# noamteyssier/ibu

Measured on AMD Instinct MI355X. Metric: records/s, fused 2-bit decode+encode of 24-byte IBU records (HBM-resident), higher is better.
Workload: dtype u64

## Files before the change

### ibu_amd/csrc/k_encode.hip

```cpp
#include "kcommon.hpp"
#include "kernels.h"

namespace ibu {

#ifndef IBU_ENCODE_MINWAVES
#define IBU_ENCODE_MINWAVES 6
#endif
#ifndef IBU_ENCODE_GEN_MINWAVES
#define IBU_ENCODE_GEN_MINWAVES 4
#endif
constexpr int encode_minwaves(int bc, int um) {
  if (bc == 0 || um == 0) return IBU_ENCODE_GEN_MINWAVES;
  return (bc <= 16 && um <= 16) ? IBU_ENCODE_MINWAVES : 4;
}
__host__ __device__ constexpr u32 enc_field_lds(int spec_len, u32 len) { return spec_len > 0 ? 128u * len : 32u * len + kStreamPad; }
template <int BC, int UM>
constexpr int enc_nt() {
#ifdef IBU_ENCODE_NT
  return (BC > 0 && UM > 0 && (BC & 3) == 0 && (UM & 3) == 0) ? IBU_ENCODE_NT : 1;
#else
  return 1;
#endif
}
#ifndef IBU_ENCODE_NT2_MINWAVES
#define IBU_ENCODE_NT2_MINWAVES 5
#endif
template <int BC, int UM>
constexpr int enc_waves() { return enc_nt<BC, UM>() > 1 ? IBU_ENCODE_NT2_MINWAVES : encode_minwaves(BC, UM); }

template <int BC, int UM, bool MSB>
__global__ void __launch_bounds__(kBlock, (enc_waves<BC, UM>()))
ibu_k_encode(const uint8_t* __restrict__ bc_in, const uint8_t* __restrict__ umi_in,
             const u64* __restrict__ idx_in, u64 first_index, u64 row_base, u32 ntiles, u32 bc_len, u32 umi_len,
             u32 wave_lds_bytes, uint8_t* __restrict__ recs, u64* __restrict__ status) {
  constexpr int NT = enc_nt<BC, UM>(), kRecs = kTileRecs * NT;
  extern __shared__ __attribute__((aligned(16))) uint8_t dyn_lds[];
  const u32 lane = threadIdx.x & (kWave - 1);
  const u32 wib = threadIdx.x >> 6;
  if (BC > 0) bc_len = BC;
  if (UM > 0) umi_len = UM;
  uint8_t* area = dyn_lds + wib * wave_lds_bytes;
  uint8_t* asc_bc = area;
  uint8_t* asc_umi = area + enc_field_lds(BC, bc_len) * NT;
  const TileRange tr = tile_range(ntiles, wib);
  const u32 nwaves = tr.stride;
  u32 t = tr.t;
  ntiles = tr.end;
  if (t >= ntiles) return;
  const uint8_t* idx_src = idx_in ? reinterpret_cast<const uint8_t*>(idx_in) + 16 * lane : bc_in;
  const size_t idx_tile = idx_in ? 1024 * NT : 0, idx_sub = idx_in ? 1024 : 0;

  AsciiStage<BC, NT> sb;
  AsciiStage<UM, NT> su;
  u32x4 vi[NT];
  sb.issue(bc_in + (size_t)t * kRecs * bc_len, bc_len, lane);
  su.issue(umi_in + (size_t)t * kRecs * umi_len, umi_len, lane);
#pragma unroll
  for (int j = 0; j < NT; ++j) vi[j] = ld16(idx_src + (size_t)t * idx_tile + j * idx_sub);
  BadRows bad;
  for (;;) {
    const size_t row0 = (size_t)t * kRecs;
    wave_lds_fence();
    const bool okcb = sb.land(asc_bc, bc_len, lane), okcu = su.land(asc_umi, umi_len, lane);
    const bool chunks_ok = okcb && okcu;
    u64 ix[NT][2];
#pragma unroll
    for (int j = 0; j < NT; ++j) {
      ix[j][0] = ((u64)vi[j].y << 32) | vi[j].x;
      ix[j][1] = ((u64)vi[j].w << 32) | vi[j].z;
      if (!idx_in) { ix[j][0] = first_index + row0 + 128 * j + 2 * lane; ix[j][1] = ix[j][0] + 1; }
    }
    const u32 tn = t + nwaves;
    const bool more = tn < ntiles;
    const u32 tp = more ? tn : t;
    sb.issue(bc_in + (size_t)tp * kRecs * bc_len, bc_len, lane);
    su.issue(umi_in + (size_t)tp * kRecs * umi_len, umi_len, lane);
#pragma unroll
    for (int j = 0; j < NT; ++j) vi[j] = ld16(idx_src + (size_t)tp * idx_tile + j * idx_sub);
    wave_lds_fence();
    u64 b[NT][2], u[NT][2];
#pragma unroll
    for (int j = 0; j < NT; ++j)
#pragma unroll
      for (int h = 0; h < 2; ++h) {
        const u32 r = 128 * j + 2 * lane + h;
        bool okb = true, oku = true;
#if IBU_PROBE == 1
        b[j][h] = *reinterpret_cast<const u32*>(asc_bc + r * bc_len);
        u[j][h] = *reinterpret_cast<const u32*>(asc_umi + r * umi_len);
#elif IBU_PROBE == 2
        b[j][h] = row0 + r;
        u[j][h] = b[j][h] * 3;
#else
        b[j][h] = pack_row<BC>(asc_bc, r, bc_len, okb);
        u[j][h] = pack_row<UM>(asc_umi, r, umi_len, oku);
        if constexpr (BC == 0 || UM == 0) {
          if (__ballot(!chunks_ok) != 0) {
            if constexpr (BC == 0) b[j][h] = pack_row_bytes(bc_in + (row0 + r) * bc_len, bc_len, okb);
            if constexpr (UM == 0) u[j][h] = pack_row_bytes(umi_in + (row0 + r) * umi_len, umi_len, oku);
          }
        }
#endif
        if (!okb) b[j][h] = 0;
        if (!oku) u[j][h] = 0;
        bad.note(!(okb && oku), row_base + row0 + r);
      }
    wave_lds_fence();
#pragma unroll
    for (int j = 0; j < NT; ++j) {
      u64* r = reinterpret_cast<u64*>(area + (128 * j + 2 * lane) * 24);
      r[0] = b[j][0]; r[1] = u[j][0]; r[2] = ix[j][0]; r[3] = b[j][1]; r[4] = u[j][1]; r[5] = ix[j][1];
    }
    wave_lds_fence();
    if constexpr (MSB) {
      rev_pairs_tile<NT>(area, 24, 0, bc_len, lane);
      rev_pairs_tile<NT>(area, 24, 8, umi_len, lane);
      wave_lds_fence();
    }
    uint8_t* dst = recs + (size_t)t * (kTileBytes * NT) + 16 * lane;
#pragma unroll
    for (int k = 0; k < 3 * NT; ++k) st16(dst + 1024 * k, *reinterpret_cast<const u32x4*>(area + 1024 * k + 16 * lane));
    if (!more) break;
    t = tn;
  }
  bad.flush(status);
}

constexpr int pack_nt(int len) { return (len > 0 && len <= 16) ? 2 : 1; }
template <int LEN, bool MSB, int GNT = 1, int RND = 0>
__global__ void __launch_bounds__(kBlock, LEN == 0 ? (RND >= 7 ? 5 : (GNT >= 4 || RND >= 5) ? 6 : 8) : LEN <= 12 ? 5 : 4)
ibu_k_pack(const uint8_t* __restrict__ in, u64 row_base, u32 ntiles , u32 len, u64* __restrict__ codes,
           u64* __restrict__ status) {
  constexpr int NT = LEN > 0 ? pack_nt(LEN) : GNT, kRows = kTileRecs * NT;
  constexpr u32 kWaveLds = LEN > 0 ? (u32)(kRows * LEN) : (u32)(256 * (RND > 0 ? RND : 4)) + kStreamPad;
  __shared__ __attribute__((aligned(16))) uint8_t lds[kWavesPerBlock * kWaveLds];
  const u32 lane = threadIdx.x & (kWave - 1);
  const u32 wib = threadIdx.x >> 6;
  uint8_t* asc = lds + wib * kWaveLds;
  const TileRange tr = tile_range(ntiles, wib);
  const u32 nwaves = tr.stride;
  u32 t = tr.t;
  ntiles = tr.end;
  if (LEN > 0) len = LEN;
  if (t >= ntiles) return;
  AsciiStage<LEN, NT, RND> sv;
  sv.issue(in + (size_t)t * kRows * len, len, lane);
  BadRows bad;
  for (;;) {
    const size_t row0 = (size_t)t * kRows;
    wave_lds_fence();
    const bool chunks_ok = sv.land(asc, len, lane);
    const u32 tn = t + nwaves;
    const bool more = tn < ntiles;
    sv.issue(in + (size_t)(more ? tn : t) * kRows * len, len, lane);
    wave_lds_fence();
#pragma unroll
    for (int j = 0; j < NT; ++j) {
      const u32 r = 128 * j + 2 * lane;
      bool ok0 = true, ok1 = true;
      u64 v0 = pack_row<LEN>(asc, r, len, ok0);
      u64 v1 = pack_row<LEN>(asc, r + 1, len, ok1);
      if constexpr (LEN == 0) {
        if (__ballot(!chunks_ok) != 0) {
          v0 = pack_row_bytes(in + (row0 + r) * len, len, ok0);
          v1 = pack_row_bytes(in + (row0 + r + 1) * len, len, ok1);
        }
      }
      if constexpr (MSB) { v0 = rev_pairs(v0, len); v1 = rev_pairs(v1, len); }
      if (!ok0) v0 = 0;
      if (!ok1) v1 = 0;
      bad.note(!ok0, row_base + row0 + r);
      bad.note(!ok1, row_base + row0 + r + 1);
      u32x4 o; o.x = (u32)v0; o.y = (u32)(v0 >> 32); o.z = (u32)v1; o.w = (u32)(v1 >> 32);
      st16(reinterpret_cast<uint8_t*>(codes) + (row0 + 128 * j) * 8 + 16 * lane, o);
    }
    if (!more) break;
    t = tn;
  }
  bad.flush(status);
}

extern "C" __global__ void ibu_k_encode_tail(const uint8_t* bc_in, const uint8_t* umi_in, const u64* idx_in,
                                             u64 first_index, u64 row0, u64 n, u32 bc_len, u32 umi_len, u32 msb,
                                             u64* __restrict__ recs, u64* status) {
  const u64 i = row0 + (u64)blockIdx.x * blockDim.x + threadIdx.x;
  if (i >= n) return;
  bool okb = true, oku = true;
  u64 b = pack_row_bytes(bc_in + i * bc_len, bc_len, okb);
  u64 u = pack_row_bytes(umi_in + i * umi_len, umi_len, oku);
  if (msb) { b = rev_pairs(b, bc_len); u = rev_pairs(u, umi_len); }
  if (!okb) b = 0;
  if (!oku) u = 0;
  if (!(okb && oku)) { atomicMin(&status[0], i); atomicAdd(&status[1], 1ull); }
  recs[3 * i] = b; recs[3 * i + 1] = u; recs[3 * i + 2] = idx_in ? idx_in[i] : first_index + i;
}
extern "C" __global__ void ibu_k_pack_tail(const uint8_t* in, u64 row0, u64 n, u32 len, u32 msb, u64* codes, u64* status) {
  const u64 i = row0 + (u64)blockIdx.x * blockDim.x + threadIdx.x;
  if (i >= n) return;
  bool ok = true;
  u64 v = pack_row_bytes(in + i * len, len, ok);
  if (msb) v = rev_pairs(v, len);
  if (!ok) { v = 0; atomicMin(&status[0], i); atomicAdd(&status[1], 1ull); }
  codes[i] = v;
}

typedef void (*EncFn)(const uint8_t*, const uint8_t*, const u64*, u64, u64, u32, u32, u32, u32, uint8_t*, u64*);
template <int B, int U, bool M>
static constexpr EncFn enc_entry() { return ibu_k_encode<len_of_mode(B), len_of_mode(U), M>; }
#define IBU_ENC_ROW(B, M) {enc_entry<B, 0, M>(), enc_entry<B, 1, M>(), enc_entry<B, 2, M>(), enc_entry<B, 3, M>(), enc_entry<B, 4, M>()}
#define IBU_ENC_TABLE(M) {IBU_ENC_ROW(0, M), IBU_ENC_ROW(1, M), IBU_ENC_ROW(2, M), IBU_ENC_ROW(3, M), IBU_ENC_ROW(4, M)}
static const EncFn kEncTable[2][kNumLenModes][kNumLenModes] = {IBU_ENC_TABLE(false), IBU_ENC_TABLE(true)};
template <int B, int U>
static constexpr int enc_nt_of() { return enc_nt<len_of_mode(B), len_of_mode(U)>(); }
#define IBU_ENC_NT_ROW(B) {enc_nt_of<B, 0>(), enc_nt_of<B, 1>(), enc_nt_of<B, 2>(), enc_nt_of<B, 3>(), enc_nt_of<B, 4>()}
static const int kEncNtTable[kNumLenModes][kNumLenModes] = {IBU_ENC_NT_ROW(0), IBU_ENC_NT_ROW(1), IBU_ENC_NT_ROW(2),
                                                            IBU_ENC_NT_ROW(3), IBU_ENC_NT_ROW(4)};

hipError_t launch_encode(const LaunchCfg& cfg, const uint8_t* bc, const uint8_t* umi, const uint64_t* idx,
                         uint64_t first_index, size_t n, uint32_t bc_len, uint32_t umi_len, void* recs,
                         uint64_t* status, hipStream_t st) {
  (void)hipGetLastError();
  if (n == 0) return hipSuccess;
  const Span sp[4] = {{recs, 24}, {bc, bc_len}, {umi, umi_len}, {idx, 8}};
  const int mb = mode_of_len(bc_len), mu = mode_of_len(umi_len);
  const u32 nt = (u32)kEncNtTable[mb][mu];
  const size_t tile_recs = (size_t)kTileRecs * nt;
  const RowSplit rs = split_rows(cfg, sp, 4, n, tile_recs);
  if (rs.head)
    hipLaunchKernelGGL(ibu_k_encode_tail, dim3(tail_grid(rs.head)), dim3(256), 0, st, bc, umi, (const u64*)idx, (u64)first_index,
                       (u64)0, (u64)rs.head, bc_len, umi_len, cfg.base_order, (u64*)recs, (u64*)status);
  if (rs.main) {
    const u32 ntiles = (u32)(rs.main / tile_recs);
    u32 wave_lds = (enc_field_lds(len_of_mode(mb), bc_len) + enc_field_lds(len_of_mode(mu), umi_len)) * nt;
    if (wave_lds < (u32)kTileBytes * nt) wave_lds = kTileBytes * nt;
    const int mo = cfg.base_order ? 1 : 0;
    const EncFn fn = kEncTable[mo][mb][mu];
    static std::atomic<int> occ[2][33][33];
    const int nb = resident_blocks<kBlock>(cfg, fn, wave_lds * kWavesPerBlock, &occ[mo][bc_len][umi_len]);
    hipLaunchKernelGGL(fn, dim3(grid_for(ntiles, cfg.cus, nb)), dim3(kBlock), wave_lds * kWavesPerBlock, st,
                       adv(bc, rs.head * bc_len), adv(umi, rs.head * umi_len), adv((const u64*)idx, 8 * rs.head),
                       (u64)(first_index + rs.head), (u64)rs.head, ntiles, bc_len, umi_len, wave_lds,
                       adv((uint8_t*)recs, 24 * rs.head), (u64*)status);
  }
  if (rs.head + rs.main < n)
    hipLaunchKernelGGL(ibu_k_encode_tail, dim3(tail_grid(n - rs.head - rs.main)), dim3(256), 0, st, bc, umi, (const u64*)idx,
                       (u64)first_index, (u64)(rs.head + rs.main), (u64)n, bc_len, umi_len, cfg.base_order, (u64*)recs, (u64*)status);
  return hipGetLastError();
}

typedef void (*PackFn)(const uint8_t*, u64, u32, u32, u64*, u64*);
#define IBU_PACK_ROW(M) {nullptr , ibu_k_pack<len_of_mode(1), M>, ibu_k_pack<len_of_mode(2), M>, \
                         ibu_k_pack<len_of_mode(3), M>, ibu_k_pack<len_of_mode(4), M>}
static const PackFn kPackTable[2][kNumLenModes] = {IBU_PACK_ROW(false), IBU_PACK_ROW(true)};
struct PackShape { int nt, rounds; };
static inline PackShape pack_shape(uint32_t len) {
  const int nt = len <= 8 ? 4 : 2;
  return {nt, (int)(len * nt + 7) / 8};
}
template <bool M>
static PackFn pack_gen_entry(int nt, int rounds) {
  switch (nt * 10 + rounds) {
    case 41: return ibu_k_pack<0, M, 4, 1>;
    case 42: return ibu_k_pack<0, M, 4, 2>;
    case 43: return ibu_k_pack<0, M, 4, 3>;
    case 44: return ibu_k_pack<0, M, 4, 4>;
    case 23: return ibu_k_pack<0, M, 2, 3>;
    case 24: return ibu_k_pack<0, M, 2, 4>;
    case 25: return ibu_k_pack<0, M, 2, 5>;
    case 26: return ibu_k_pack<0, M, 2, 6>;
    case 27: return ibu_k_pack<0, M, 2, 7>;
    default: return ibu_k_pack<0, M, 2, 8>;
  }
}

hipError_t launch_pack(const LaunchCfg& cfg, const uint8_t* in, size_t n, uint32_t len, uint64_t* codes,
                       uint64_t* status, hipStream_t st) {
  (void)hipGetLastError();
  if (n == 0) return hipSuccess;
  const Span sp[2] = {{in, len}, {codes, 8}};
  const int m = mode_of_len(len), mo = cfg.base_order ? 1 : 0;
  const PackShape shape = m ? PackShape{pack_nt(len_of_mode(m)), 0} : pack_shape(len);
  const size_t tile_rows = (size_t)kTileRecs * shape.nt;
  const RowSplit rs = split_rows(cfg, sp, 2, n, tile_rows);
  if (rs.head)
    hipLaunchKernelGGL(ibu_k_pack_tail, dim3(tail_grid(rs.head)), dim3(256), 0, st, in, (u64)0, (u64)rs.head, len, cfg.base_order,
                       (u64*)codes, (u64*)status);
  if (rs.main) {
    const u32 ntiles = (u32)(rs.main / tile_rows);
    const PackFn fn = m ? kPackTable[mo][m] : (mo ? pack_gen_entry<true>(shape.nt, shape.rounds) : pack_gen_entry<false>(shape.nt, shape.rounds));
    static std::atomic<int> occ[2][kNumLenModes], occ_gen[2][33];
    std::atomic<int>* oc = m ? &occ[mo][m] : &occ_gen[mo][len];
    hipLaunchKernelGGL(fn, dim3(grid_for(ntiles, cfg.cus, resident_blocks<kBlock>(cfg, fn, 0, oc))),
                       dim3(kBlock), 0, st, adv(in, rs.head * len), (u64)rs.head, ntiles, len, adv((u64*)codes, 8 * rs.head),
                       (u64*)status);
  }
  if (rs.head + rs.main < n)
    hipLaunchKernelGGL(ibu_k_pack_tail, dim3(tail_grid(n - rs.head - rs.main)), dim3(256), 0, st, in, (u64)(rs.head + rs.main),
                       (u64)n, len, cfg.base_order, (u64*)codes, (u64*)status);
  return hipGetLastError();
}

}
```

### ibu_amd/csrc/kcommon.hpp

```cpp
#pragma once
#include <hip/hip_runtime.h>
#include <stdint.h>
#include <stdio.h>
#include <stdlib.h>

#include "kernels.h"

namespace ibu {

typedef unsigned int u32;
typedef unsigned long long u64;
typedef u32 u32x4 __attribute__((ext_vector_type(4)));
typedef u32 u32x2 __attribute__((ext_vector_type(2)));

static constexpr int kWave = 64;
#ifndef IBU_BLOCK
#define IBU_BLOCK 256
#endif
static constexpr int kBlock = IBU_BLOCK;
static constexpr int kWavesPerBlock = kBlock / kWave;
static constexpr int kTileRecs = 128;
static constexpr int kTileBytes = kTileRecs * 24;
static constexpr u32 kPool = 0x54474341u;

static constexpr int kNumLenModes = 5;
__host__ __device__ constexpr int len_of_mode(int m) { return m == 1 ? 8 : m == 2 ? 12 : m == 3 ? 16 : m == 4 ? 32 : 0; }
static inline int mode_of_len(uint32_t len) {
  switch (len) {
    case 8: return 1;
    case 12: return 2;
    case 16: return 3;
    case 32: return 4;
    default: return 0;
  }
}

#ifndef IBU_XCD_REMAP
#define IBU_XCD_REMAP 1
#endif
__device__ __forceinline__ u32 logical_block() {
#if IBU_XCD_REMAP
  const u32 nb = gridDim.x;
  if (nb & 7u) return blockIdx.x;
  return (blockIdx.x & 7u) * (nb >> 3) + (blockIdx.x >> 3);
#else
  return blockIdx.x;
#endif
}

#ifndef IBU_XCD_STATIC
#define IBU_XCD_STATIC 1
#endif
struct TileRange { u32 t, stride, end; };
#ifndef IBU_XCD_SUB
#define IBU_XCD_SUB 1
#endif
__device__ __forceinline__ TileRange tile_range(u32 ntiles, u32 wib) {
#if IBU_XCD_STATIC
  if ((gridDim.x & 7u) == 0 && gridDim.x >= 8u * IBU_XCD_SUB) {
    const u32 parts = 8u * IBU_XCD_SUB;
    const u32 tpp = (ntiles + parts - 1) / parts;
    const u32 xcd = blockIdx.x & 7u, lb = blockIdx.x >> 3, nbx = gridDim.x >> 3;
    const u32 sub = lb % IBU_XCD_SUB, part = xcd * IBU_XCD_SUB + sub;
    const u32 nb_sub = (nbx - sub + IBU_XCD_SUB - 1) / IBU_XCD_SUB;
    const u32 t0 = part * tpp, t1 = t0 + tpp < ntiles ? t0 + tpp : ntiles;
    return {t0 + (lb / IBU_XCD_SUB) * (u32)kWavesPerBlock + wib, nb_sub * (u32)kWavesPerBlock, t0 < ntiles ? t1 : 0u};
  }
#endif
  return {logical_block() * (u32)kWavesPerBlock + wib, gridDim.x * (u32)kWavesPerBlock, ntiles};
}

template <class Regs, class Load, class Body>
__device__ __forceinline__ void sweep_tiles(const TileRange tr, Load load, Body body) {
  u32 t = tr.t;
  if (t >= tr.end) return;
  Regs a, b;
  load(a, t);
  for (;;) {
    u32 tn = t + tr.stride;
    bool more = tn < tr.end;
    load(b, more ? tn : t);
    body(a, t);
    if (!more) break;
    t = tn;
    tn = t + tr.stride;
    more = tn < tr.end;
    load(a, more ? tn : t);
    body(b, t);
    if (!more) break;
    t = tn;
  }
}

#ifndef IBU_NT_LOAD
#define IBU_NT_LOAD 1
#endif
#ifndef IBU_NT_STORE
#define IBU_NT_STORE 1
#endif
#ifndef IBU_ST_POLICY
#define IBU_ST_POLICY 0
#endif
#ifndef IBU_LD_POLICY
#define IBU_LD_POLICY 0
#endif
struct WaveBuf {
  __amdgpu_buffer_rsrc_t r;
  u32 voff;
  __device__ __forceinline__ explicit WaveBuf(const void* p) {
    const u64 a = (u64)p;
    const u64 first = ((u64)(u32)__builtin_amdgcn_readfirstlane((u32)(a >> 32)) << 32) | (u64)(u32)__builtin_amdgcn_readfirstlane((u32)a);
    const u64 base = first - (1ull << 30);
    r = __builtin_amdgcn_make_buffer_rsrc(reinterpret_cast<void*>(base), 0, -1, 0x00020000);
    voff = (u32)(a - base);
  }
};
__device__ __forceinline__ u32x4 ld16(const void* p) {
#if IBU_LD_POLICY
  const WaveBuf w(p);
  return __builtin_amdgcn_raw_buffer_load_b128(w.r, (int)w.voff, 0, IBU_LD_POLICY - 1);
#elif IBU_NT_LOAD
  return __builtin_nontemporal_load(reinterpret_cast<const u32x4*>(p));
#else
  return *reinterpret_cast<const u32x4*>(p);
#endif
}
__device__ __forceinline__ void st16(void* p, u32x4 v) {
#if IBU_ST_POLICY
  const WaveBuf w(p);
  __builtin_amdgcn_raw_buffer_store_b128(v, w.r, (int)w.voff, 0, IBU_ST_POLICY - 1);
#elif IBU_NT_STORE
  __builtin_nontemporal_store(v, reinterpret_cast<u32x4*>(p));
#else
  *reinterpret_cast<u32x4*>(p) = v;
#endif
}

__device__ __forceinline__ void wave_lds_fence() {
  __builtin_amdgcn_fence(__ATOMIC_RELEASE, "wavefront");
  __builtin_amdgcn_wave_barrier();
  __builtin_amdgcn_fence(__ATOMIC_ACQUIRE, "wavefront");
}

__device__ __forceinline__ u64 rev_pairs(u64 x, u32 len) {
  u64 r = __builtin_bitreverse64(x);
  r = ((r >> 1) & 0x5555555555555555ull) | ((r & 0x5555555555555555ull) << 1);
  return r >> (64 - 2 * len);
}
__device__ __forceinline__ u32x4 rev_pairs_x2(u32x4 v, u32 len) {
  const u64 a = rev_pairs(((u64)v.y << 32) | v.x, len), b = rev_pairs(((u64)v.w << 32) | v.z, len);
  u32x4 o; o.x = (u32)a; o.y = (u32)(a >> 32); o.z = (u32)b; o.w = (u32)(b >> 32);
  return o;
}
template <int NT = 1>
__device__ __forceinline__ void rev_pairs_tile(uint8_t* tile, u32 rstride, u32 foff, u32 len, u32 lane) {
#pragma unroll
  for (int j = 0; j < NT; ++j)
#pragma unroll
    for (int h = 0; h < 2; ++h) {
      u64* p = reinterpret_cast<u64*>(tile + (size_t)(128 * j + 2 * lane + h) * rstride + foff);
      *p = rev_pairs(*p, len);
    }
}

__device__ __forceinline__ u32 expand4(u32 x) {
  u32 t = (x | (x << 12)) & 0x000F000Fu;
  t = (t | (t << 6)) & 0x03030303u;
  return __builtin_amdgcn_perm(kPool, kPool, t);
}
__device__ __forceinline__ u32 pack4(u32 w, bool& ok) {
  u32 sel = ((w >> 1) ^ (w >> 2)) & 0x03030303u;
  u32 expect = __builtin_amdgcn_perm(kPool, kPool, sel);
  ok = ok && ((w & 0xDFDFDFDFu) == expect);
  u32 y = sel | (sel >> 6);
  return (y | (y >> 12)) & 0xFFu;
}
__device__ __forceinline__ u32 pack1(u32 c, bool& ok) {
  u32 code = ((c >> 1) ^ (c >> 2)) & 3u;
  ok = ok && ((c & 0xDFu) == ((kPool >> (8 * code)) & 0xFFu));
  return code;
}
__device__ __forceinline__ u32x4 expand16(u32 w) {
  u32x4 o;
  o.x = expand4(w & 0xFF); o.y = expand4((w >> 8) & 0xFF);
  o.z = expand4((w >> 16) & 0xFF); o.w = expand4(w >> 24);
  return o;
}

#ifndef IBU_PROBE
#define IBU_PROBE 0
#endif
__device__ __forceinline__ u32x4 expand_chunk(const uint8_t* tile, u32 rstride, u32 foff, u32 len, u32 c) {
#if IBU_PROBE == 1
  { const u32 w = *reinterpret_cast<const u32*>(tile + (c & 127u) * rstride + foff); u32x4 o; o.x = o.y = o.z = o.w = w; return o; }
#elif IBU_PROBE == 2
  { u32x4 o; o.x = o.y = o.z = o.w = c + len + rstride + foff; return o; }
#endif
  const u32 l4 = len >> 2;
  if (l4 == 4) return expand16(*reinterpret_cast<const u32*>(tile + c * rstride + foff));
  if (l4 == 8) return expand16(*reinterpret_cast<const u32*>(tile + (c >> 1) * rstride + foff + (c & 1) * 4));
  const u32 d = 4 * c;
  u32 r = (d * (65536u / l4 + 1)) >> 16;
  u32 q = d - r * l4;
  u32 v[4];
#pragma unroll
  for (int j = 0; j < 4; ++j) {
    v[j] = expand4(tile[r * rstride + foff + q]);
    if (++q == l4) { q = 0; ++r; }
  }
  u32x4 o; o.x = v[0]; o.y = v[1]; o.z = v[2]; o.w = v[3];
  return o;
}

__host__ __device__ __forceinline__ u64 splitmix64(u64 z) {
  z += 0x9E3779B97F4A7C15ull;
  z = (z ^ (z >> 30)) * 0xBF58476D1CE4E5B9ull;
  z = (z ^ (z >> 27)) * 0x94D049BB133111EBull;
  return z ^ (z >> 31);
}
__device__ __forceinline__ u64 mask2(u32 len) { return len >= 32 ? ~0ull : ((1ull << (2 * len)) - 1); }

static constexpr u32 kStreamPad = 16;
__host__ __device__ constexpr u32 stream_bytes(int nt) { return 1024u * nt + kStreamPad; }

#ifndef IBU_STREAM_PROBE
#define IBU_STREAM_PROBE 0
#endif
__device__ __forceinline__ void lds_or(u32* p, u32 v) {
#if IBU_STREAM_PROBE == 1
  *p = v;
#else
  (void)__hip_atomic_fetch_or(p, v, __ATOMIC_RELAXED, __HIP_MEMORY_SCOPE_WAVEFRONT);
#endif
}
template <int NT>
__device__ __forceinline__ void stream_from_rows(const uint8_t* tile, u32 rstride, u32 foff, u32 len, u32* stream, u32 lane) {
#if IBU_STREAM_PROBE == 2
  return;
#endif
  u32x4 z; z.x = z.y = z.z = z.w = 0;
#pragma unroll
  for (int k = 0; k < NT; ++k) *reinterpret_cast<u32x4*>(reinterpret_cast<uint8_t*>(stream) + 1024 * k + 16 * lane) = z;
  if (lane == 0) *reinterpret_cast<u32x4*>(reinterpret_cast<uint8_t*>(stream) + 1024 * NT) = z;
  wave_lds_fence();
  const u64 m = mask2(len);
  const bool wide = len > 16;
#pragma unroll
  for (int j = 0; j < NT; ++j)
#pragma unroll
    for (int h = 0; h < 2; ++h) {
      const u32 r = 128 * j + 2 * lane + h;
      const u64 v = *reinterpret_cast<const u64*>(tile + (size_t)r * rstride + foff) & m;
      const u32 bit = r * 2 * len, s = bit & 31u;
      u32* d = stream + (bit >> 5);
      const u64 t = v << s;
      lds_or(d, (u32)t);
      lds_or(d + 1, (u32)(t >> 32));
      if (wide) lds_or(d + 2, (u32)((v >> 32) >> (32 - s)));
    }
  wave_lds_fence();
}
template <int NT>
__device__ __forceinline__ void expand_stream(const u32* stream, u32 len, uint8_t* out_tile, u32 lane) {
  const u32 nchunks = 8 * len * NT;
#pragma unroll
  for (int i = 0; i < 4 * NT; ++i) {
    const u32 c = lane + 64 * i;
    if (c < nchunks) st16(out_tile + 16 * (size_t)c, expand16(stream[c]));
  }
}
__device__ __forceinline__ u64 stream_row(const u32* stream, u32 r, u32 len) {
  const u32 bit = r * 2 * len, s = bit & 31u;
  const u32* d = stream + (bit >> 5);
  const u32 w0 = d[0], w1 = d[1], w2 = d[2];
  const u32 lo = __builtin_amdgcn_alignbit(w1, w0, s), hi = __builtin_amdgcn_alignbit(w2, w1, s);
  return (((u64)hi << 32) | lo) & mask2(len);
}

template <int LEN, int NT = 1>
__device__ __forceinline__ void expand_field(const uint8_t* tile, u32 rstride, u32 foff, u32 rt_len,
                                             uint8_t* out_tile, u32 lane, u32* stream = nullptr) {
  static_assert((LEN & 3) == 0, "specialised lengths are multiples of 4");
  if constexpr (LEN > 0) {
    constexpr u32 last = 8 * LEN * NT - 1;
    constexpr int rounds = (8 * LEN * NT + kWave - 1) / kWave;
#pragma unroll
    for (int i = 0; i < rounds; ++i) {
      u32 c = lane + 64 * i;
      c = c < last ? c : last;
      st16(out_tile + 16 * (size_t)c, expand_chunk(tile, rstride, foff, (u32)LEN, c));
    }
  } else {
    stream_from_rows<NT>(tile, rstride, foff, rt_len, stream, lane);
    expand_stream<NT>(stream, rt_len, out_tile, lane);
  }
}

template <int L4>
__device__ __forceinline__ u64 pack_row_dwords(const uint8_t* row, bool& ok) {
  u64 v = 0;
#pragma unroll
  for (int q = 0; q < L4; ++q) v |= (u64)pack4(*reinterpret_cast<const u32*>(row + 4 * q), ok) << (8 * q);
  return v;
}
__device__ __forceinline__ u64 pack_row_bytes(const uint8_t* row, u32 len, bool& ok) {
  u64 v = 0;
  for (u32 i = 0; i < len; ++i) v |= (u64)pack1(row[i], ok) << (2 * i);
  return v;
}
template <int LEN>
__device__ __forceinline__ u64 pack_row(const uint8_t* field, u32 r, u32 rt_len, bool& ok) {
  if constexpr (LEN > 0 && (LEN & 3) == 0) {
    return pack_row_dwords<LEN / 4>(field + r * LEN, ok);
  } else {
    static_assert(LEN == 0, "specialised lengths are multiples of 4; every other length is a runtime length");
    return stream_row(reinterpret_cast<const u32*>(field), r, rt_len);
  }
}

template <int LEN, int NT = 1, int RND = 0>
struct AsciiStage {
  static constexpr int rounds = LEN > 0 ? (LEN * NT + 7) / 8 : (RND > 0 ? RND : 4);
  u32x4 v[rounds];
  __device__ __forceinline__ void issue(const uint8_t* g, u32 rt_len, u32 lane) {
    const u32 last = 8 * (LEN > 0 ? (u32)(LEN * NT) : rt_len * NT) - 1;
#pragma unroll
    for (int i = 0; i < rounds; ++i) {
      u32 c = lane + 64 * i;
      c = c < last ? c : last;
      v[i] = ld16(g + 16 * (size_t)c);
    }
  }
  __device__ __forceinline__ bool land(uint8_t* lds, u32 rt_len, u32 lane) const {
    const u32 nchunks = 8 * (LEN > 0 ? (u32)(LEN * NT) : rt_len * NT);
    bool ok = true;
#pragma unroll
    for (int i = 0; i < rounds; ++i) {
      const u32 c = lane + 64 * i;
      if constexpr (LEN > 0) {
        if (c < nchunks) *reinterpret_cast<u32x4*>(lds + 16 * c) = v[i];
      } else {
        if (64u * i < nchunks) {
          bool okc = true;
          const u32 w = pack4(v[i].x, okc) | (pack4(v[i].y, okc) << 8) | (pack4(v[i].z, okc) << 16) | (pack4(v[i].w, okc) << 24);
          if (c < nchunks) { reinterpret_cast<u32*>(lds)[c] = w; ok = ok && okc; }
        }
      }
    }
    return ok;
  }
};

struct BadRows {
  u64 first = ~0ull;
  u32 count = 0;
  __device__ __forceinline__ void note(bool bad, u64 row_global) {
    if (bad) { first = row_global < first ? row_global : first; ++count; }
  }
  __device__ __forceinline__ void flush(u64* status) const {
    if (__ballot(count != 0) == 0) return;
    u64 f = first;
    u32 c = count;
#pragma unroll
    for (int m = 32; m >= 1; m >>= 1) {
      const u32 flo = __shfl_xor((u32)f, m), fhi = __shfl_xor((u32)(f >> 32), m);
      const u64 fo = ((u64)fhi << 32) | flo;
      f = fo < f ? fo : f;
      c += __shfl_xor(c, m);
    }
    if ((threadIdx.x & (kWave - 1)) == 0) { atomicMin(&status[0], f); atomicAdd(&status[1], (u64)c); }
  }
};


static inline u32 grid_for(u32 ntiles, int cus, int blocks_per_cu) {
  u32 need = (ntiles + kWavesPerBlock - 1) / kWavesPerBlock;
  u32 cap = (u32)(cus * blocks_per_cu);
  return need < cap ? (need ? need : 1) : cap;
}
static inline bool aligned16(const void* p) { return (reinterpret_cast<uintptr_t>(p) & 15u) == 0; }

struct Span { const void* p; size_t stride; };
static inline int peel_rows(const Span* s, int k) {
  for (int h = 0; h < 16; ++h) {
    bool ok = true;
    for (int i = 0; i < k; ++i)
      if (s[i].p && ((reinterpret_cast<uintptr_t>(s[i].p) + (uintptr_t)h * s[i].stride) & 15u)) ok = false;
    if (ok) return h;
  }
  return -1;
}
struct RowSplit { size_t head, main; };
static inline RowSplit split_rows(const LaunchCfg& cfg, const Span* s, int k, size_t n, size_t tile) {
  const int h = peel_rows(s, k);
  RowSplit rs{n, 0};
  if (h >= 0) {
    rs.head = (size_t)h < n ? (size_t)h : n;
    rs.main = ((n - rs.head) / tile) * tile;
  }
  if (cfg.trace_rows) fprintf(stderr, "ibu rows: n=%zu head=%zu tiled=%zu rest=%zu tile=%zu\n", n, rs.head, rs.main, n - rs.head - rs.main, tile);
  return rs;
}
template <class T> static inline T* adv(T* p, size_t bytes) {
  return p ? reinterpret_cast<T*>(reinterpret_cast<uintptr_t>(p) + bytes) : p;
}
static inline u32 tail_grid(u64 rows) { return (u32)((rows + 255) / 256); }
static inline u32 capped_grid(const LaunchCfg& cfg, u64 items, u64 per_block, u32 blocks_per_cu = 8) {
  u64 blocks = (items + per_block - 1) / per_block;
  const u64 cap = (u64)cfg.cus * blocks_per_cu;
  if (blocks > cap) blocks = cap;
  return (u32)(blocks ? blocks : 1);
}

__device__ __forceinline__ u64 shfl_xor64(u64 v, int m) {
  u32 lo = __shfl_xor((u32)v, m), hi = __shfl_xor((u32)(v >> 32), m);
  return ((u64)hi << 32) | lo;
}
__device__ __forceinline__ u64 shfl_up64(u64 v, int d) {
  u32 lo = __shfl_up((u32)v, d), hi = __shfl_up((u32)(v >> 32), d);
  return ((u64)hi << 32) | lo;
}
__device__ __forceinline__ u32 shfl_xor_lanes(u32 v, int m) { return __shfl_xor(v, m); }
__device__ __forceinline__ u64 shfl_xor_lanes(u64 v, int m) { return shfl_xor64(v, m); }
__device__ __forceinline__ u32 shfl_up_lanes(u32 v, int d) { return __shfl_up(v, d); }
__device__ __forceinline__ u64 shfl_up_lanes(u64 v, int d) { return shfl_up64(v, d); }
struct OpAdd { template <class T> __device__ __forceinline__ T operator()(T a, T b) const { return a + b; } };
struct OpMin { template <class T> __device__ __forceinline__ T operator()(T a, T b) const { return b < a ? b : a; } };
template <class T, class Op>
__device__ __forceinline__ T wave_reduce(T v, Op op) {
#pragma unroll
  for (int m = 32; m >= 1; m >>= 1) v = op(v, shfl_xor_lanes(v, m));
  return v;
}
template <class T, int K, class Op>
__device__ __forceinline__ void wave_reduce(T (&v)[K], Op op) {
#pragma unroll
  for (int m = 32; m >= 1; m >>= 1)
#pragma unroll
    for (int k = 0; k < K; ++k) v[k] = op(v[k], shfl_xor_lanes(v[k], m));
}
template <class T, class Op>
__device__ __forceinline__ T wave_scan(T v, Op op) {
  const u32 lane = threadIdx.x & (kWave - 1);
#pragma unroll
  for (int d = 1; d < kWave; d <<= 1) {
    const T front = shfl_up_lanes(v, d);
    if (lane >= (u32)d) v = op(front, v);
  }
  return v;
}

__device__ __forceinline__ u32 block_exclusive_scan(u32 v, u32* wsum , u32* total) {
  const u32 lane = threadIdx.x & (kWave - 1), wib = threadIdx.x >> 6;
  const u32 inc = wave_scan(v, OpAdd{});
  if (lane == kWave - 1 && wib < 4) wsum[wib] = inc;
  __syncthreads();
  u32 off = 0, tot = 0;
#pragma unroll
  for (int w = 0; w < 4; ++w) {
    const u32 s = wsum[w];
    if ((u32)w < wib) off += s;
    tot += s;
  }
  __syncthreads();
  *total = tot;
  return off + inc - v;
}

}
```

Measured before the change: 51.35 billion.

## Pack chunk-aligned fields directly into record tile instead of ASCII staging

For fixed field lengths of 8, 16 or 32 bases, the loaded ASCII chunks are packed to 2-bit codes while landing and written straight into the 24-byte record slots in LDS. This skips the separate ASCII staging area and the per-row repack pass for those fields. Invalid rows fall back to a rolled per-byte repack from global memory. LDS use per wave changes: a tile area plus any remaining staging, which can raise or lower occupancy depending on the length combination.

Result: no change. 51.08 billion (-0.5%).

```diff
diff --git a/ibu_amd/csrc/k_encode.hip b/ibu_amd/csrc/k_encode.hip
--- a/ibu_amd/csrc/k_encode.hip
+++ b/ibu_amd/csrc/k_encode.hip
@@ -28,20 +28,36 @@
 template <int BC, int UM>
 constexpr int enc_waves() { return enc_nt<BC, UM>() > 1 ? IBU_ENCODE_NT2_MINWAVES : encode_minwaves(BC, UM); }
 
+#ifndef IBU_ENC_CHUNK
+#define IBU_ENC_CHUNK 1
+#endif
+__host__ __device__ constexpr bool enc_direct(int bc, int um) {
+  return IBU_ENC_CHUNK > 1 || (bc == 32 && (um == 32 || um == 16 || um == 12)) || (bc == 16 && um == 32);
+}
+__host__ __device__ constexpr bool enc_chunked(int len, int bc, int um) {
+  return IBU_ENC_CHUNK && IBU_PROBE == 0 && chunk_len(len) && enc_direct(bc, um);
+}
+__host__ __device__ constexpr u32 enc_wave_lds(int bc, int um, u32 bc_len, u32 umi_len, u32 nt) {
+  const bool cb = enc_chunked(bc, bc, um), cu = enc_chunked(um, bc, um);
+  const u32 stage = ((cb ? 0u : enc_field_lds(bc, bc_len)) + (cu ? 0u : enc_field_lds(um, umi_len))) * nt, tile = (u32)kTileBytes * nt;
+  return (cb || cu) ? tile + stage : (stage > tile ? stage : tile);
+}
+
 template <int BC, int UM, bool MSB>
 __global__ void __launch_bounds__(kBlock, (enc_waves<BC, UM>()))
 ibu_k_encode(const uint8_t* __restrict__ bc_in, const uint8_t* __restrict__ umi_in,
              const u64* __restrict__ idx_in, u64 first_index, u64 row_base, u32 ntiles, u32 bc_len, u32 umi_len,
              u32 wave_lds_bytes, uint8_t* __restrict__ recs, u64* __restrict__ status) {
   constexpr int NT = enc_nt<BC, UM>(), kRecs = kTileRecs * NT;
+  constexpr bool CB = enc_chunked(BC, BC, UM), CU = enc_chunked(UM, BC, UM), kDirect = CB || CU;
   extern __shared__ __attribute__((aligned(16))) uint8_t dyn_lds[];
   const u32 lane = threadIdx.x & (kWave - 1);
   const u32 wib = threadIdx.x >> 6;
   if (BC > 0) bc_len = BC;
   if (UM > 0) umi_len = UM;
   uint8_t* area = dyn_lds + wib * wave_lds_bytes;
-  uint8_t* asc_bc = area;
-  uint8_t* asc_umi = area + enc_field_lds(BC, bc_len) * NT;
+  uint8_t* asc_bc = area + (kDirect ? kTileBytes * NT : 0);
+  uint8_t* asc_umi = asc_bc + (CB ? 0 : enc_field_lds(BC, bc_len) * NT);
   const TileRange tr = tile_range(ntiles, wib);
   const u32 nwaves = tr.stride;
   u32 t = tr.t;
@@ -61,7 +77,9 @@
   for (;;) {
     const size_t row0 = (size_t)t * kRecs;
     wave_lds_fence();
-    const bool okcb = sb.land(asc_bc, bc_len, lane), okcu = su.land(asc_umi, umi_len, lane);
+    bool okcb, okcu;
+    if constexpr (CB) okcb = sb.land_codes(area, 24, 0, lane); else okcb = sb.land(asc_bc, bc_len, lane);
+    if constexpr (CU) okcu = su.land_codes(area, 24, 8, lane); else okcu = su.land(asc_umi, umi_len, lane);
     const bool chunks_ok = okcb && okcu;
     u64 ix[NT][2];
 #pragma unroll
@@ -78,6 +96,35 @@
 #pragma unroll
     for (int j = 0; j < NT; ++j) vi[j] = ld16(idx_src + (size_t)tp * idx_tile + j * idx_sub);
     wave_lds_fence();
+    if constexpr (kDirect) {
+      const bool redo = __ballot(!chunks_ok) != 0;
+#pragma unroll
+      for (int j = 0; j < NT; ++j)
+#pragma unroll
+        for (int h = 0; h < 2; ++h) {
+          const u32 r = 128 * j + 2 * lane + h;
+          u64* rec = reinterpret_cast<u64*>(area + r * 24);
+          bool okb = true, oku = true;
+          if constexpr (!CB) {
+            u64 b = pack_row<BC>(asc_bc, r, bc_len, okb);
+            if constexpr (BC == 0) { if (redo) b = pack_row_bytes(bc_in + (row0 + r) * bc_len, bc_len, okb); }
+            rec[0] = okb ? b : 0;
+          } else if (redo) {
+            (void)pack_row_bytes_rolled(bc_in + (row0 + r) * bc_len, bc_len, okb);
+            if (!okb) rec[0] = 0;
+          }
+          if constexpr (!CU) {
+            u64 u = pack_row<UM>(asc_umi, r, umi_len, oku);
+            if constexpr (UM == 0) { if (redo) u = pack_row_bytes(umi_in + (row0 + r) * umi_len, umi_len, oku); }
+            rec[1] = oku ? u : 0;
+          } else if (redo) {
+            (void)pack_row_bytes_rolled(umi_in + (row0 + r) * umi_len, umi_len, oku);
+            if (!oku) rec[1] = 0;
+          }
+          rec[2] = ix[j][h];
+          bad.note(!(okb && oku), row_base + row0 + r);
+        }
+    } else {
     u64 b[NT][2], u[NT][2];
 #pragma unroll
     for (int j = 0; j < NT; ++j)
@@ -110,6 +157,7 @@
     for (int j = 0; j < NT; ++j) {
       u64* r = reinterpret_cast<u64*>(area + (128 * j + 2 * lane) * 24);
       r[0] = b[j][0]; r[1] = u[j][0]; r[2] = ix[j][0]; r[3] = b[j][1]; r[4] = u[j][1]; r[5] = ix[j][1];
+    }
     }
     wave_lds_fence();
     if constexpr (MSB) {
@@ -231,8 +279,7 @@
                        (u64)0, (u64)rs.head, bc_len, umi_len, cfg.base_order, (u64*)recs, (u64*)status);
   if (rs.main) {
     const u32 ntiles = (u32)(rs.main / tile_recs);
-    u32 wave_lds = (enc_field_lds(len_of_mode(mb), bc_len) + enc_field_lds(len_of_mode(mu), umi_len)) * nt;
-    if (wave_lds < (u32)kTileBytes * nt) wave_lds = kTileBytes * nt;
+    const u32 wave_lds = enc_wave_lds(len_of_mode(mb), len_of_mode(mu), bc_len, umi_len, nt);
     const int mo = cfg.base_order ? 1 : 0;
     const EncFn fn = kEncTable[mo][mb][mu];
     static std::atomic<int> occ[2][33][33];
diff --git a/ibu_amd/csrc/kcommon.hpp b/ibu_amd/csrc/kcommon.hpp
--- a/ibu_amd/csrc/kcommon.hpp
+++ b/ibu_amd/csrc/kcommon.hpp
@@ -308,6 +308,12 @@
   for (u32 i = 0; i < len; ++i) v |= (u64)pack1(row[i], ok) << (2 * i);
   return v;
 }
+__device__ __forceinline__ u64 pack_row_bytes_rolled(const uint8_t* row, u32 len, bool& ok) {
+  u64 v = 0;
+#pragma clang loop unroll(disable)
+  for (u32 i = 0; i < len; ++i) v |= (u64)pack1(row[i], ok) << (2 * i);
+  return v;
+}
 template <int LEN>
 __device__ __forceinline__ u64 pack_row(const uint8_t* field, u32 r, u32 rt_len, bool& ok) {
   if constexpr (LEN > 0 && (LEN & 3) == 0) {
@@ -318,6 +324,7 @@
   }
 }
 
+__host__ __device__ constexpr bool chunk_len(int len) { return len == 8 || len == 16 || len == 32; }
 template <int LEN, int NT = 1, int RND = 0>
 struct AsciiStage {
   static constexpr int rounds = LEN > 0 ? (LEN * NT + 7) / 8 : (RND > 0 ? RND : 4);
@@ -349,8 +356,25 @@
     }
     return ok;
   }
+  __device__ __forceinline__ bool land_codes(uint8_t* tile, u32 rstride, u32 foff, u32 lane) const {
+    static_assert(chunk_len(LEN), "8, 16 or 32 bases: every round is whole, every lane writes");
+    bool ok = true;
+#pragma unroll
+    for (int i = 0; i < rounds; ++i) {
+      const u32 c = lane + 64 * i;
+      const u32 w = pack4(v[i].x, ok) | (pack4(v[i].y, ok) << 8) | (pack4(v[i].z, ok) << 16) | (pack4(v[i].w, ok) << 24);
+      if constexpr (LEN == 16) {
+        *reinterpret_cast<u64*>(tile + c * rstride + foff) = w;
+      } else if constexpr (LEN == 32) {
+        *reinterpret_cast<u32*>(tile + (c >> 1) * rstride + foff + 4 * (c & 1)) = w;
+      } else {
+        *reinterpret_cast<u64*>(tile + 2 * c * rstride + foff) = w & 0xFFFFu;
+        *reinterpret_cast<u64*>(tile + (2 * c + 1) * rstride + foff) = w >> 16;
+      }
+    }
+    return ok;
+  }
 };
-
 struct BadRows {
   u64 first = ~0ull;
   u32 count = 0;
```
